# IvanIZ/BenchPush

Hardware: AMD Instinct MI355X
Metric: env-steps/sec at N=4096 envs (ship-ice-v0), 1/2/4/8 MI355X (higher is better)
Workload: dtype f64

## Files before the change

### __graft_entry__.py

```python
import os
import subprocess
import sys

ROOT = os.path.dirname(os.path.abspath(__file__))
if ROOT not in sys.path:
    sys.path.insert(0, ROOT)


def build():
    from benchpush_amd.build import build_debug_paths, build_hip
    build_hip(force=True, verbose=True)
    build_debug_paths(force=True, verbose=True)
    subprocess.check_call(["make", "-C", os.path.join(ROOT, "oracle")])
    import benchpush_amd
    from benchpush_amd import _lib
    L = _lib.load()
    for name in _lib.EXPORTS:
        getattr(L, name)
    assert L.bp_abi_version() == 11


def smoke():
    import numpy as np
    import torch

    from benchpush_amd.envs.ship_ice import BatchedShipIceEnv, default_trials
    from oracle.oracle import OracleShipIce

    trials = default_trials(0.3, 2, base_seed=7)
    env = BatchedShipIceEnv(4, cfg={"concentration": 0.3}, trials=trials, device="cuda:0")
    obs, info = env.reset()
    cfg = env.cfg
    orcs = [OracleShipIce(env.params, cfg.ship.vertices, cfg.ship.head, cfg.ship.tail) for _ in range(4)]
    oobs = [o.reset(trials[e % 2])[0] for e, o in enumerate(orcs)]
    assert all(np.array_equal(obs[e].cpu().numpy(), oobs[e]) for e in range(4)), "reset observation differs from oracle"
    rng = np.random.default_rng(0)
    for t in range(2):
        a = rng.uniform(-1, 1, 4).astype(np.float32).astype(np.float64)
        obs, rew, term, trunc, info = env.step(torch.from_numpy(a))
        bs = env.body_state().cpu().numpy()
        for e, o in enumerate(orcs):
            oo, orr, ot, oi = o.step(float(a[e]))
            nb = len(o.bodies())
            assert np.array_equal(bs[e, :nb], o.bodies()), "body state differs from oracle"
            assert np.array_equal(obs[e].cpu().numpy(), oo), "observation differs from oracle"
            assert float(rew[e]) == orr and bool(term[e]) == ot, "reward/termination differs from oracle"
    env.check_errors()
    env.close()
    from benchpush_amd import box_delivery_scenario as S
    from benchpush_amd.envs.box_delivery import BatchedBoxDeliveryEnv
    from oracle.oracle_bd import BD_INFO_KEYS, OracleBoxDelivery

    benv = BatchedBoxDeliveryEnv(2, num_trials=2, device="cuda:0")
    bobs, _ = benv.reset()
    borc = []
    for e in range(2):
        o = OracleBoxDelivery(S.box_delivery_physics_params(benv.cfg), dict(benv.bd_params), benv.cfg)
        assert np.array_equal(bobs[e].cpu().numpy(), o.reset(benv.trials[e])), "box-delivery reset observation differs from oracle"
        borc.append(o)
    acts = np.array([0.4, -0.7])
    bobs, brew, bterm, btrunc, binfo = benv.step(torch.from_numpy(acts))
    for e, o in enumerate(borc):
        oo, orr, ot, otr, oi = o.step(float(acts[e]))
        assert np.array_equal(bobs[e].cpu().numpy(), oo) and float(brew[e]) == orr, "box-delivery step differs from oracle"
        assert np.array_equal(binfo[e].cpu().numpy(), np.array([oi[k] for k in BD_INFO_KEYS])), "box-delivery info differs from oracle"
    benv.check_errors()
    benv.close()
    print("smoke ok: ship-ice 4 envs x 2 steps and box-delivery 2 envs x 1 step bit-identical to the oracles")


if __name__ == "__main__":
    build()
    if len(sys.argv) > 1 and sys.argv[1] == "smoke":
        smoke()
```

### benchpush_amd/build.py

```python
import os
import subprocess

_HERE = os.path.dirname(os.path.abspath(__file__))
CSRC = os.path.join(_HERE, "csrc")
LIB_PATH = os.path.join(_HERE, "libbenchpush_hip.so")
SOURCES = ["bp_capi.hip"]


def _headers():
    import glob
    return sorted(glob.glob(os.path.join(CSRC, "*.hpp"))) + [os.path.join(_HERE, "..", "include", "benchpush_amd.h")]

HIPCC_FLAGS = ["--offload-arch=gfx950", "-O3", "-ffp-contract=off", "-fno-fast-math", "-fPIC", "-shared", "-std=c++17",
               "-Wno-unused-value"]


def needs_build():
    if not os.path.exists(LIB_PATH):
        return True
    t = os.path.getmtime(LIB_PATH)
    for p in [os.path.join(CSRC, f) for f in SOURCES] + _headers():
        if os.path.exists(p) and os.path.getmtime(p) > t:
            return True
    return False


def build_hip(force=False, verbose=False):
    if not force and not needs_build():
        return LIB_PATH
    hipcc = os.environ.get("HIPCC", "/opt/rocm/bin/hipcc")
    if not os.path.exists(hipcc):
        hipcc = "hipcc"
    cmd = [hipcc] + HIPCC_FLAGS + ["-o", LIB_PATH] + [os.path.join(CSRC, s) for s in SOURCES]
    if verbose:
        print(" ".join(cmd))
    subprocess.check_call(cmd, cwd=CSRC)
    return LIB_PATH


DBG_LIB_PATH = os.path.join(_HERE, "libbenchpush_hip_dbgpaths.so")


def build_debug_paths(force=False, verbose=False):
    if not force and os.path.exists(DBG_LIB_PATH):
        t = os.path.getmtime(DBG_LIB_PATH)
        if all(os.path.getmtime(p) <= t for p in [os.path.join(CSRC, f) for f in SOURCES] + _headers() if os.path.exists(p)):
            return DBG_LIB_PATH
    hipcc = os.environ.get("HIPCC", "/opt/rocm/bin/hipcc")
    if not os.path.exists(hipcc):
        hipcc = "hipcc"
    cmd = [hipcc] + HIPCC_FLAGS + ["-DBP_DEBUG_PATHS=1", "-o", DBG_LIB_PATH] + [os.path.join(CSRC, s) for s in SOURCES]
    if verbose:
        print(" ".join(cmd))
    subprocess.check_call(cmd, cwd=CSRC)
    return DBG_LIB_PATH


if __name__ == "__main__":
    print(build_hip(force=True, verbose=True))
    print(build_debug_paths(force=True, verbose=True))
```

### benchpush_amd/csrc/bp_capi.hip

```cpp
#include <hip/hip_runtime.h>

#include <cstdio>
#include <cstdlib>
#include <algorithm>
#include <cstring>
#include <map>
#include <mutex>
#include <string>
#include <vector>

#include <fcntl.h>
#include <sys/file.h>
#include <sys/stat.h>
#include <unistd.h>

#include "bp_host_bd.hpp"
#include "bp_boxdelivery.hpp"
#include "bp_policy.hpp"
#include "bp_render.hpp"

struct bp_handle {
    bp_config cfg;
    int num_envs = 0;
    long long env_offset = 0;
// ... 134 lines not shown
        L.fd = open(key.c_str(), O_RDWR | O_CREAT | O_CLOEXEC, 0666);
        umask(um);
        if (L.fd < 0) { g_res_locks.erase(key); return; }
        (void)flock(L.fd, LOCK_SH);
    }
    L.refs++;
    h->dev_lock_key = key;
}
static void resident_release(bp_handle *h)
{
    if (h->dev_lock_key.empty()) return;
    std::lock_guard<std::mutex> g(g_res_mu);
    auto it = g_res_locks.find(h->dev_lock_key);
    if (it != g_res_locks.end() && --it->second.refs <= 0) { close(it->second.fd); g_res_locks.erase(it); }
    h->dev_lock_key.clear();
}
static bool resident_device_shared(bp_handle *h)
{
    if (h->dev_lock_key.empty()) return false;
    std::lock_guard<std::mutex> g(g_res_mu);
    auto it = g_res_locks.find(h->dev_lock_key);
    if (it == g_res_locks.end()) return false;
    if (flock(it->second.fd, LOCK_EX | LOCK_NB) == 0) { (void)flock(it->second.fd, LOCK_SH); return false; }
    (void)flock(it->second.fd, LOCK_SH);
    return true;
}
static int device_cus(bp_handle *h)
{
    if (h->num_cus <= 0) {
        hipDeviceProp_t prop;
        HIPCHK(h, hipGetDeviceProperties(&prop, h->device));
        h->num_cus = prop.multiProcessorCount;
    }
    return BP_OK;
}
static int sched_persist_setup(bp_handle *h)
{
    int rc = device_cus(h);
    if (rc) return rc;
    const int slots = h->num_cus * 4 * (h->P.env_kind == BP_ENV_SHIP_ICE ? BP_SCHED_WAVES : 2);
    const int pers = getenv("BP_SCHED_PERSIST") ? atoi(getenv("BP_SCHED_PERSIST")) : 1;
    h->sched_persist = pers > 0 ? std::min(h->num_envs, slots * pers) : 0;
    if (h->sched_persist && !h->pd_buf) HIPCHK(h, hipMalloc(&h->pd_buf, sizeof(DevParams) + sizeof(DevPtrs)));
    if (h->sched_persist && !getenv("BP_SCHED_PERSIST")) {
        h->resident_auto = true;
        resident_acquire(h);
        h->device_shared = resident_device_shared(h);
    }
    return BP_OK;
}
extern "C" {

int32_t bp_abi_version(void) { return BP_ABI_VERSION; }
int32_t bp_sizeof_config(void) { return (int32_t)sizeof(bp_config); }

const char *bp_last_error(const bp_handle *h) { return h ? h->err.c_str() : "null handle"; }

int bp_create(const bp_config *cfg, int32_t num_envs, int64_t env_id_offset, int32_t device, bp_handle **out)
{
    if (!cfg || !out || num_envs <= 0) return BP_EINVAL;
    *out = nullptr;
    int ndev = 0;
    if (hipGetDeviceCount(&ndev) != hipSuccess || ndev <= 0 || device < 0 || device >= ndev) return BP_ENODEVICE;
    if (!(cfg->damping_pow >= 0.0) || cfg->damping_pow > 1.0) return BP_EINVAL;
    if (cfg->num_ship_verts < 3 || cfg->num_ship_verts > BP_MAX_SHIP_VERTS) return BP_EINVAL;
    if (cfg->steps <= 0 || cfg->iterations <= 0 || cfg->persistence <= 0) return BP_EINVAL;
    if (cfg->env_kind != BP_ENV_SHIP_ICE && cfg->env_kind != BP_ENV_MAZE) return BP_EINVAL;
    if (cfg->env_kind == BP_ENV_MAZE && (cfg->num_wheels < 0 || cfg->num_wheels > BP_MAX_WHEELS)) return BP_EINVAL;
    if (cfg->random_start && cfg->env_kind != BP_ENV_SHIP_ICE) return BP_EINVAL;
    bp_handle *h = new bp_handle();
    h->cfg = *cfg;
    h->num_envs = num_envs;
    h->env_offset = env_id_offset;
    h->device = device;
    h->resettle = (cfg->env_kind == BP_ENV_SHIP_ICE && cfg->random_start != 0);
    DevGuard _dg(device);
    if (!_dg.ok) { delete h; return BP_ENODEVICE; }
    memset(&h->D, 0, sizeof(h->D));
    DevParams &P = h->P;
    memset(&P, 0, sizeof(P));
    P.dt_sub = cfg->dt / cfg->steps;
    P.steps = cfg->steps; P.iterations = cfg->iterations; P.persistence = cfg->persistence; P.settle_steps = cfg->settle_steps;
    if (const char *evp = getenv("BP_DEBUG_PATHS")) P.dbg_paths = atoi(evp);
    P.damping_pow = cfg->damping_pow; P.bias_coef = cfg->bias_coef; P.slop = cfg->slop;
    P.target_speed = cfg->target_speed; P.max_yaw_rate = cfg->max_yaw_rate;
    P.map_w = cfg->map_w; P.map_h = cfg->map_h; P.goal_y = cfg->goal_y; P.m_to_pix = cfg->m_to_pix;
    P.beta = cfg->beta; P.boundary_penalty = cfg->boundary_penalty; P.terminal_reward = cfg->terminal_reward;
    P.local_w = cfg->local_w; P.local_h = cfg->local_h; P.vshift = cfg->vshift; P.obs_range = cfg->obs_range;
    P.skin = 0.06;
    P.env_kind = cfg->env_kind;
    P.nkin = (cfg->env_kind == BP_ENV_MAZE) ? 1 + cfg->num_wheels : 1;
    P.goal_x = cfg->goal_x; P.goal_reach = cfg->goal_reach; P.k_increment = cfg->k_increment;
    P.num_envs = num_envs; P.env_offset = env_id_offset;
    P.random_start = (cfg->env_kind == BP_ENV_SHIP_ICE) ? cfg->random_start : 0;
    P.start_x_range = cfg->start_x_range; P.start_seed = cfg->start_seed; P.ship_mass = cfg->ship_mass;
    P.num_ship_verts = cfg->num_ship_verts;
    memcpy(P.ship_verts, cfg->ship_verts, sizeof(P.ship_verts));
    memcpy(P.ship_head, cfg->ship_head, sizeof(P.ship_head));
    memcpy(P.ship_tail, cfg->ship_tail, sizeof(P.ship_tail));
    const double grid = 1.0 / cfg->m_to_pix;
    P.grid_w = (int)(cfg->map_w / grid);
    P.grid_h = (int)(cfg->map_h / grid);
    P.obs_h = (int)(cfg->local_h * cfg->m_to_pix);
    P.obs_w = (int)(cfg->local_w * cfg->m_to_pix);
    if ((P.obs_h * P.obs_w) % 4 != 0) { delete h; return BP_EINVAL; }
    if (cfg->env_kind == BP_ENV_MAZE) {
        const int infl = (P.obs_w > P.obs_h ? P.obs_w : P.obs_h) / 2;
        const int nwords = ((P.obs_h + infl) * (P.obs_w + infl) + 31) / 32;
        h->obs_lds_bytes = (size_t)4 * (nwords + ((nwords + 1) & ~1)) + sizeof(double) * 2 * MZ_MAXBOX * 4;
        if (hipFuncSetAttribute((const void *)k_observe_maze, hipFuncAttributeMaxDynamicSharedMemorySize, (int)h->obs_lds_bytes) != hipSuccess) { delete h; return BP_EHIP; }
    } else {
        if (P.obs_h % 2 != 0 || P.obs_w % 2 != 0 || P.obs_w / 2 > OBS_THREADS_SHIP) { delete h; return BP_EINVAL; }
        h->obs_lds_bytes = (size_t)((P.obs_h * P.obs_w + 15) & ~15) + (size_t)((P.obs_h + 15) & ~15) + sizeof(double) * 2 * OBS_CHUNK * BP_MAXV;
        if (hipFuncSetAttribute((const void *)k_observe, hipFuncAttributeMaxDynamicSharedMemorySize, (int)h->obs_lds_bytes) != hipSuccess) { delete h; return BP_EHIP; }
    }
    *out = h;
    return BP_OK;
}

int bp_destroy(bp_handle *h)
{
    if (!h) return BP_EINVAL;
    DevGuard _dg(h->device);
    if (h->st_aux) { hipStreamSynchronize(h->st_aux); hipStreamDestroy(h->st_aux); }
    resident_release(h);
    if (h->pd_buf) hipFree(h->pd_buf);
    if (h->st_aux2) { hipStreamSynchronize(h->st_aux2); hipStreamDestroy(h->st_aux2); }
    if (h->st_aux3) { hipStreamSynchronize(h->st_aux3); hipStreamDestroy(h->st_aux3); }
    if (h->ev_join3) hipEventDestroy(h->ev_join3);
    for (hipStream_t s_ : h->st_parts) { hipStreamSynchronize(s_); hipStreamDestroy(s_); }
    for (hipEvent_t e_ : h->ev_parts) hipEventDestroy(e_);
    if (h->ev_join2) hipEventDestroy(h->ev_join2);
    if (h->ev_fork) hipEventDestroy(h->ev_fork);
    if (h->ev_join) hipEventDestroy(h->ev_join);
    for (void *p : h->allocs) hipFree(p);
    for (hipEvent_t e : h->ev) hipEventDestroy(e);
    delete h;
    return BP_OK;
}

static int upload_trials(bp_handle *h, const std::vector<std::vector<bpgeom::Shape>> &trials, bool settle = true)
{
    using namespace bpgeom;
    const int T = (int)trials.size();
    int maxnb = 1;
    for (const auto &b : trials) maxnb = std::max(maxnb, (int)b.size());
    if (maxnb > 60000) return fail(h, BP_EINVAL, "too many bodies");
    const int nbcap = (maxnb + 7) / 8 * 8;
    h->nbcap = nbcap;
    h->num_trials = T;
    h->P.nbcap = nbcap;
    h->P.mvcap = mvcap_for(nbcap);
    h->P.num_trials = T;
    h->lds_bytes = lds_bytes_for(nbcap, h->P.env_kind == BP_ENV_BOX);
    if (h->lds_bytes > 160 * 1024) return fail(h, BP_EINVAL, "nb_cap too large for LDS");
    if (nbcap >= (1 << BP_CC_IDX_BITS)) return fail(h, BP_EINVAL, "nb_cap exceeds the candidate cache's body-index field (16384 bodies per env)");

    std::vector<int> h_nb(T), h_nv((size_t)T * nbcap, 0), h_kind((size_t)T * nbcap, 0);
    std::vector<d2> h_lv((size_t)T * nbcap * BP_MAXV), h_ln((size_t)T * nbcap * BP_MAXV);
    std::vector<double4> h_mass((size_t)T * nbcap), h_pose((size_t)T * nbcap), h_prop((size_t)T * nbcap);
    memset(h_lv.data(), 0, h_lv.size() * sizeof(d2));
    memset(h_ln.data(), 0, h_ln.size() * sizeof(d2));
    memset(h_mass.data(), 0, h_mass.size() * sizeof(double4));
    memset(h_pose.data(), 0, h_pose.size() * sizeof(double4));
    memset(h_prop.data(), 0, h_prop.size() * sizeof(double4));
    for (int t = 0; t < T; t++) {
// ... 833 lines not shown
{
    if (!h || !mask || !src || !dst || rows < 0 || row_bytes <= 0 || (row_bytes & 3) != 0 || rows > 0x7FFFFFFF) return BP_EINVAL;
    if ((((size_t)src) | ((size_t)dst)) & 3) return BP_EINVAL;
    BP_DEVICE(h);
    if (rows == 0) return BP_OK;
    hipLaunchKernelGGL(k_copy_rows_masked, dim3((unsigned)rows), dim3(256), 0, (hipStream_t)stream, (const unsigned char *)mask, (const unsigned *)src,
                       (unsigned *)dst, (long long)(row_bytes / 4));
    HIPCHK(h, hipGetLastError());
    return BP_OK;
}

int bp_debug_round2(const double *in_dev, double *out_dev, int32_t n, void *stream)
{
    if (!in_dev || !out_dev || n < 0) return BP_EINVAL;
    hipLaunchKernelGGL(k_debug_round2, dim3((n + 255) / 256), dim3(256), 0, (hipStream_t)stream, in_dev, out_dev, n);
    return hipGetLastError() == hipSuccess ? BP_OK : BP_EHIP;
}

int bp_get_body_state(bp_handle *h, double *out, void *stream)
{
    if (!h || !out) return BP_EINVAL;
    if (!h->loaded || !h->was_reset) return fail(h, BP_ESTATE, "not reset");
    BP_DEVICE(h);
    hipLaunchKernelGGL(k_export_bodies, dim3(h->num_envs), dim3(256), 0, (hipStream_t)stream, h->P, h->D, out);
    HIPCHK(h, hipGetLastError());
    return BP_OK;
}
int bp_costmap_update(bp_handle *h, const bp_costmap_config *cfg, const double *ship_pos_y, double vs, double *out, void *stream)
{
    if (!h || !cfg || !out) return BP_EINVAL;
    if (!h->loaded || !h->was_reset) return fail(h, BP_ESTATE, "bp_costmap_update before bp_load_scenarios/bp_reset");
    if (h->P.env_kind != BP_ENV_SHIP_ICE) return fail(h, BP_EINVAL, "bp_costmap_update: ship-ice handles only");
    const int H = (int)(cfg->m * cfg->scale), W = (int)(cfg->n * cfg->scale);
    if (!(cfg->scale > 0) || H <= 0 || W <= 0 || cfg->margin < 0 || 2 * cfg->margin > W) return fail(h, BP_EINVAL, "bp_costmap_update: bad grid");
    BP_DEVICE(h);
    hipStream_t st = (hipStream_t)stream;
    const size_t total = (size_t)h->num_envs * H * W;
    const int nblk = (int)std::min<size_t>((total + 255) / 256, 65535);
    hipLaunchKernelGGL(k_costmap_init, dim3(nblk), dim3(256), 0, st, out, h->num_envs, H, W, (int)cfg->margin);
    const int groups = (h->P.nbcap - h->P.nkin + 3) / 4;
    if (groups > 0)
        hipLaunchKernelGGL(k_costmap, dim3(h->num_envs, groups), dim3(256), 0, st, h->P, h->D, cfg->scale, H, W, cfg->alpha, cfg->ship_mass,
                           cfg->horizon > 0 ? cfg->horizon * cfg->scale : 0.0, ship_pos_y, vs, out);
    HIPCHK(h, hipGetLastError());
    return BP_OK;
}
int bp_get_low_dim_obs(bp_handle *h, double *out, void *stream)
{
    if (!h || !out) return BP_EINVAL;
    if (!h->loaded || !h->was_reset) return fail(h, BP_ESTATE, "not reset");
    BP_DEVICE(h);
    hipLaunchKernelGGL(k_export_lowdim, dim3(h->num_envs), dim3(256), 0, (hipStream_t)stream, h->P, h->D, out);
    HIPCHK(h, hipGetLastError());
    return BP_OK;
}

int32_t bp_nb_cap(const bp_handle *h) { return h ? h->nbcap : 0; }
int32_t bp_obs_height(const bp_handle *h) { return h ? h->P.obs_h : 0; }
int32_t bp_obs_width(const bp_handle *h) { return h ? h->P.obs_w : 0; }

int32_t bp_bd_sizeof_config(void) { return (int32_t)sizeof(bp_bd_config); }

int bp_bd_create(const bp_bd_config *cfg, int32_t num_envs, int64_t env_id_offset, int32_t device, bp_handle **out)
{
    if (!cfg || !out || num_envs <= 0) return BP_EINVAL;
    *out = nullptr;
    int ndev = 0;
    if (hipGetDeviceCount(&ndev) != hipSuccess || ndev <= 0 || device < 0 || device >= ndev) return BP_ENODEVICE;
    if (!(cfg->damping_pow >= 0.0) || cfg->damping_pow > 1.0 || cfg->steps <= 0 || cfg->iterations <= 0 || cfg->persistence <= 0) return BP_EINVAL;
    if (cfg->num_boxes <= 0 || cfg->num_boxes > BD_MAXBOX || cfg->local_px <= 0 || (cfg->local_px & 1)) return BP_EINVAL;
    bp_handle *h = new bp_handle();
    memset(&h->cfg, 0, sizeof(h->cfg));
    h->bdcfg = *cfg;
    h->num_envs = num_envs; h->env_offset = env_id_offset; h->device = device;
    DevGuard _dg(device);
    if (!_dg.ok) { delete h; return BP_ENODEVICE; }
    memset(&h->D, 0, sizeof(h->D));
    memset(&h->Q, 0, sizeof(h->Q));
    DevParams &P = h->P;
    memset(&P, 0, sizeof(P));
    P.dt_sub = cfg->ctrl_dt / cfg->steps;
    P.steps = cfg->steps; P.iterations = cfg->iterations; P.persistence = cfg->persistence; P.settle_steps = cfg->settle_steps;
    if (const char *evp = getenv("BP_DEBUG_PATHS")) P.dbg_paths = atoi(evp);
    P.damping_pow = cfg->damping_pow; P.bias_coef = cfg->bias_coef; P.slop = cfg->slop;
    P.target_speed = cfg->target_speed;
    P.skin = 0.25;
    P.env_kind = BP_ENV_BOX;
    P.nkin = 6;
    P.num_envs = num_envs; P.env_offset = env_id_offset;
    P.obs_h = P.obs_w = cfg->local_px;
    BdParams &B = h->B;
    memset(&B, 0, sizeof(B));
    B.room_length = cfg->room_length; B.room_width = cfg->room_width; B.recept_x = cfg->recept_x; B.recept_y = cfg->recept_y;
    B.recept_size = cfg->recept_size; B.ppm = cfg->ppm; B.local_w = cfg->local_w; B.robot_radius = cfg->robot_radius;
    B.step_size = cfg->step_size; B.target_speed = cfg->target_speed; B.ctrl_dt = cfg->ctrl_dt;
    B.partial_rewards_scale = cfg->partial_rewards_scale; B.goal_reward = cfg->goal_reward; B.collision_penalty = cfg->collision_penalty;
    B.non_movement_penalty = cfg->non_movement_penalty; B.correct_direction_reward_scale = cfg->correct_direction_reward_scale;
    B.ministep_size = cfg->ministep_size; B.sp_channel_scale = cfg->sp_channel_scale;
    B.local_px = cfg->local_px; B.use_correct_direction_reward = cfg->use_correct_direction_reward;
    B.inactivity_cutoff = cfg->inactivity_cutoff; B.num_boxes = cfg->num_boxes; B.step_limit = cfg->step_limit;
    B.first_box = 6;
    B.action_type = cfg->action_type;
    if (cfg->action_type < 0 || cfg->action_type > 2) { delete h; return BP_EINVAL; }
    B.task = cfg->task; B.omega_scale = cfg->omega_scale; B.v_scale = cfg->v_scale; B.lfc = cfg->lfc;
    B.yaw_rate_step = cfg->yaw_rate_step; B.t_max = cfg->t_max;
    B.boundary_penalty = cfg->boundary_penalty; B.box_cleared_reward = cfg->box_cleared_reward; B.box_putback_penalty = cfg->box_putback_penalty;
    B.truncation_penalty = cfg->truncation_penalty; B.terminal_reward = cfg->terminal_reward; B.pushing_mult = cfg->pushing_mult;
    B.recept_outside = (cfg->task == 0 && cfg->invert_receptacle_map) ? 1.0f : 0.0f;
    if (cfg->task == 1) {
        if (cfg->num_boundary_verts < 3 || cfg->num_boundary_verts > 8 || cfg->num_outer_verts < 3 || cfg->num_outer_verts > 8 ||
            cfg->num_goal_points < 1 || cfg->num_goal_points > 128) { delete h; return BP_EINVAL; }
        B.nbd = cfg->num_boundary_verts; B.nob = cfg->num_outer_verts; B.ngoal = cfg->num_goal_points;
        memcpy(B.bd_poly, cfg->boundary, sizeof(B.bd_poly)); memcpy(B.ob_poly, cfg->outer_boundary, sizeof(B.ob_poly));
        memcpy(B.footprint, cfg->footprint_verts, sizeof(B.footprint));
        B.recept_outside = 1.0f;
    } else if (cfg->task != 0) { delete h; return BP_EINVAL; }
    *out = h;
    return BP_OK;
}

int bp_bd_load(bp_handle *h, int32_t T, int32_t nbox, const double *starts, const double *boxes, int32_t ns, const double *sverts,
               const int32_t *scount, const double *spose, const double *srad, const int32_t *stype)
{
    if (!h || T <= 0 || nbox <= 0 || nbox > BD_MAXBOX || ns <= 0 || !starts || !boxes || !sverts || !scount || !spose || !srad || !stype) return BP_EINVAL;
    if (h->loaded) return fail(h, BP_ESTATE, "scenarios already loaded");
    if (h->P.env_kind != BP_ENV_BOX) return fail(h, BP_ESTATE, "handle was created for another environment");
    BP_DEVICE(h);
    using namespace bpgeom;
    const bp_bd_config &cf = h->bdcfg;
    std::vector<std::vector<Shape>> trials(T);
    std::vector<Shape> recepts(T);
    h->bd_map_of_trial.assign(T, 0);
    std::vector<std::vector<std::vector<P2>>> map_keys;
    int nphys_static = -1;
    for (int t = 0; t < T; t++) {
        std::vector<Shape> &bodies = trials[t];
        const double sx = starts[3 * t], sy = starts[3 * t + 1], sh = starts[3 * t + 2];
        {
            Shape s;
            build_agent_main(cf.robot_verts, 4, sx, sy, sh, s);
            s.radius = 0.0; s.e = 0.01; s.u = 1.0; s.kind = kind_of(1, 1, BODY_KINEMATIC);
            bodies.push_back(s);
            for (int k = 0; k < 5; k++) {
                Shape w;
                build_kinematic_part(k < 4 ? cf.wheel_verts[k] : cf.bumper_verts, 4, sx, sy, sh, w);
                w.radius = 0.02; w.e = 0.01; w.u = 0.0; w.kind = kind_of(0, 1, BODY_KINEMATIC);
                bodies.push_back(w);
            }
        }
        for (int b = 0; b < nbox; b++) {
            const double *bx = boxes + ((size_t)t * nbox + b) * 3;
            Shape s;
            if (!build_box(bx[0], bx[1], bx[2], cf.box_half, cf.box_density, 0.02, s)) return fail(h, BP_EINVAL, "degenerate box");
            s.radius = 0.02; s.e = 0.01; s.u = 1.0; s.kind = kind_of(2, 0, BODY_DYNAMIC);
            bodies.push_back(s);
        }
        std::vector<std::vector<P2>> obstacles;
        int nrec = 0, nst = 0;
        for (int k = 0; k < ns; k++) {
            const size_t o = (size_t)t * ns + k;
            const int n = scount[o];
            if (n == 0) continue;
            if (n < 3 || n > 4) return fail(h, BP_EINVAL, "static polygons have 3 or 4 vertices");
            Shape s;
            build_static_poly(sverts + o * 8, n, spose[o * 3], spose[o * 3 + 1], spose[o * 3 + 2], s);
            s.radius = srad[o]; s.e = 0.01; s.u = 1.0;
// ... 462 lines not shown
```

### benchpush_amd/csrc/bp_device.hpp

```cpp
#pragma once
#include <hip/hip_runtime.h>
#include <stdint.h>

#include "../../include/benchpush_amd.h"

#define BP_KADJ 24
#define BP_ACAP 64

typedef double2 d2;

enum { BODY_DYNAMIC = 0, BODY_KINEMATIC = 1, BODY_STATIC = 2 };
__device__ __forceinline__ int kind_ctype(int k) { return k & 0xFF; }
__device__ __forceinline__ int kind_group(int k) { return (k >> 8) & 0xFF; }
__device__ __forceinline__ int kind_btype(int k) { return (k >> 16) & 3; }
enum { ARB_FIRST = 0, ARB_NORMAL = 1, ARB_IGNORE = 2, ARB_CACHED = 3 };
#define ARB_FREE_KEY 0xFFFFFFFFu

struct DevParams {
    double dt_sub;
    int steps, iterations, persistence, settle_steps;
    double damping_pow, bias_coef, slop, target_speed, max_yaw_rate, map_w, map_h, goal_y, m_to_pix;
    double beta, boundary_penalty, terminal_reward, local_w, local_h, vshift, obs_range;
    double goal_x, goal_reach, k_increment;
    int env_kind;
    int nkin;
    double skin;
    int nbcap, mvcap, num_envs, num_trials, num_ship_verts;
    long long env_offset;
    double ship_verts[BP_MAX_SHIP_VERTS][2];
    double ship_head[2], ship_tail[2];
    int obs_h, obs_w, grid_h, grid_w;
    int sq_chunk, sq_levels, sq_cap;
    int sq_cls;
    unsigned sq_ymask;
    int sq_dynprio;
    int sq_parts, sq_part;
    int sq_floor;
    int sq_lrpt, sq_bw, sq_hyst;
    int sq_hold;
    int sq_mode;
    int sq_image;
    unsigned sq_img_lds;
    unsigned sq_img_stride;
    int sq_debug;
    int dbg_paths;
    int pair_mode, pair_solo;
    int pp_max_keys, pp_max_slots, pp_max_mv, pp_max_act, pp_max_work;
    int pp_snake, pp_heavy_only;
    int pp_rate;
    int random_start;
    double start_x_range, ship_mass;
    unsigned long long start_seed;
};

struct DevPtrs {
    const int *sc_nb;
    const int *sc_nv;
    const d2 *sc_lv;
    const d2 *sc_ln;
    const double4 *sc_mass;
    const double4 *sc_pose;
    const double4 *sc_prop;
    const int *sc_kind;
    const double *dist_map;
    const unsigned char *wall_map;
    const double *goal_raw;
    const double *maze_obs_map;
    int *e_trial, *e_episode, *e_nb, *e_err;
    int *e_flags;
    double *e_prevdist;
    unsigned *e_stamp;
    double *e_currdt, *e_total_work, *e_ke, *e_imp;
    unsigned *e_cnt;
    unsigned *e_cost;
    const int *order;
    int *sq_items;
    int *sq_ctr;
    unsigned *sq_carry;
    unsigned char *sq_moved;
    unsigned char *sq_img;
    int *sq_done;
    int *sq_lev;
    unsigned *sq_thr;
    int *sq_sub;
    int *sq_pairstat;
    int *sq_rescue;
    int *sq_warn;
    d2 *pxy;
    double *ang;
    d2 *rot;
    d2 *velv, *velw, *velb;
    d2 *wv, *wn, *pv;
    double4 *bb, *fat;
    unsigned short *adj;
    unsigned char *adjn;
    unsigned long long *hint;
    unsigned *a_key, *a_stamp, *a_sc, *a_h0, *a_h1;
    double *a_d;
    double *e_lastrew;
    int *e_lastflag;
    double *m_acc;
    double *m_rows;
    double *m_ring;
    double *m_sum;
    unsigned *m_count;
    unsigned char *m_open;
    unsigned long long *clk;
    double *dbg;
    int dbg_env;
    unsigned long long *prof;
};

__device__ __forceinline__ d2 mk2(double x, double y) { d2 r; r.x = x; r.y = y; return r; }
__device__ __forceinline__ double vdot(d2 a, d2 b) { return a.x * b.x + a.y * b.y; }
__device__ __forceinline__ double vcross(d2 a, d2 b) { return a.x * b.y - a.y * b.x; }
__device__ __forceinline__ d2 vsub(d2 a, d2 b) { return mk2(a.x - b.x, a.y - b.y); }
__device__ __forceinline__ d2 vadd(d2 a, d2 b) { return mk2(a.x + b.x, a.y + b.y); }
__device__ __forceinline__ d2 vneg(d2 a) { return mk2(-a.x, -a.y); }
__device__ __forceinline__ d2 vmul(d2 a, double s) { return mk2(a.x * s, a.y * s); }
__device__ __forceinline__ d2 vperp(d2 a) { return mk2(-a.y, a.x); }
__device__ __forceinline__ d2 vrotate(d2 a, d2 b) { return mk2(a.x * b.x - a.y * b.y, a.x * b.y + a.y * b.x); }
__device__ __forceinline__ double vlen(d2 a) { return __builtin_sqrt(vdot(a, a)); }
__device__ __forceinline__ d2 vlerp(d2 a, d2 b, double t) { return vadd(vmul(a, 1.0 - t), vmul(b, t)); }
__device__ __forceinline__ double clamp01(double f) { return fmax(0.0, fmin(f, 1.0)); }
__device__ __forceinline__ double fclampd(double f, double lo, double hi) { return fmin(fmax(f, lo), hi); }

#define HW_PLANE_A(h) ((int)((h) & 31ull))
// ... 92 lines not shown
__device__ __forceinline__ void bp_sincos(double x, double &sn, double &cs)
{
    const double invpio2 = 6.36619772367581382433e-01;
    const double pio2_1 = 1.57079632673412561417e+00, pio2_1t = 6.07710050650619224932e-11;
    const double pio2_2 = 6.07710050630396597660e-11, pio2_2t = 2.02226624879595063154e-21;
    const double S1 = -1.66666666666666324348e-01, S2 = 8.33333333332248946124e-03, S3 = -1.98412698298579493134e-04,
                 S4 = 2.75573137070700676789e-06, S5 = -2.50507602534068634195e-08, S6 = 1.58969099521155010221e-10;
    const double C1 = 4.16666666666666019037e-02, C2 = -1.38888888888741095749e-03, C3 = 2.48015872894767294178e-05,
                 C4 = -2.75573143513906633035e-07, C5 = 2.08757232129817482790e-09, C6 = -1.13596475577881948265e-11;
    double fn = __builtin_rint(x * invpio2);
    double r = x - fn * pio2_1;
    double w = fn * pio2_1t;
    double y0 = r - w;
    const bool deep = __builtin_fabs(y0) < __builtin_fabs(x) * 7.62939453125e-06;
    if (__builtin_expect(__ballot(deep) != 0ull, 0)) {
        const double t = r;
        const double w2 = fn * pio2_2;
        const double r2 = t - w2;
        const double w3 = fn * pio2_2t - ((t - r2) - w2);
        if (deep) { r = r2; w = w3; y0 = r2 - w3; }
    }
    double y1 = (r - y0) - w;
    int q = (int)((long long)fn & 3);
    double z = y0 * y0;
    double v = z * y0;
    double rs = S2 + z * (S3 + z * (S4 + z * (S5 + z * S6)));
    double ks = y0 - ((z * (0.5 * y1 - v * rs) - y1) - v * S1);
    double rc = z * (C1 + z * (C2 + z * (C3 + z * (C4 + z * (C5 + z * C6)))));
    double kc = 1.0 - (0.5 * z - (z * rc - y0 * y1));
    const bool odd = (q & 1) != 0;
    const double s0 = odd ? kc : ks, c0 = odd ? ks : kc;
    const int sflip = (q & 2) ? (int)0x80000000 : 0, cflip = ((q + 1) & 2) ? (int)0x80000000 : 0;
    sn = __hiloint2double(__double2hiint(s0) ^ sflip, __double2loint(s0));
    cs = __hiloint2double(__double2hiint(c0) ^ cflip, __double2loint(c0));
}

__host__ __device__ inline unsigned long long bp_splitmix64(unsigned long long x)
{
    x += 0x9E3779B97F4A7C15ull;
    x = (x ^ (x >> 30)) * 0xBF58476D1CE4E5B9ull;
    x = (x ^ (x >> 27)) * 0x94D049BB133111EBull;
    return x ^ (x >> 31);
}
__host__ __device__ inline double bp_start_u01(unsigned long long seed, long long gid, long long episode)
{
    const unsigned long long k = bp_splitmix64(seed ^ bp_splitmix64(((unsigned long long)gid << 32) + (unsigned long long)episode));
    return (double)(k >> 11) * (1.0 / 9007199254740992.0);
}

__device__ __forceinline__ int lane_id() { return (int)(threadIdx.x & 63); }
__device__ __forceinline__ unsigned long long ballot(bool p) { return __ballot(p); }
__device__ __forceinline__ int popc_below(unsigned long long m, int lane) { return __popcll(m & ((1ull << lane) - 1ull)); }

template <int CTRL>
__device__ __forceinline__ double dpp_mov_f64(double v)
{
    int lo = __double2loint(v), hi = __double2hiint(v);
    lo = __builtin_amdgcn_update_dpp(lo, lo, CTRL, 0xF, 0xF, false);
    hi = __builtin_amdgcn_update_dpp(hi, hi, CTRL, 0xF, 0xF, false);
    return __hiloint2double(hi, lo);
}
__device__ __forceinline__ double half_max(double v)
{
    v = fmax(v, dpp_mov_f64<0xB1>(v));
    v = fmax(v, dpp_mov_f64<0x4E>(v));
    v = fmax(v, dpp_mov_f64<0x141>(v));
    v = fmax(v, dpp_mov_f64<0x140>(v));
    v = fmax(v, __shfl_xor(v, 16));
    return v;
}
__device__ __forceinline__ double half_min(double v)
{
    v = fmin(v, dpp_mov_f64<0xB1>(v));
    v = fmin(v, dpp_mov_f64<0x4E>(v));
    v = fmin(v, dpp_mov_f64<0x141>(v));
    v = fmin(v, dpp_mov_f64<0x140>(v));
    v = fmin(v, __shfl_xor(v, 16));
    return v;
}
__device__ __forceinline__ double readlane_f64(double v, int l)
{
    return __hiloint2double(__builtin_amdgcn_readlane(__double2hiint(v), l), __builtin_amdgcn_readlane(__double2loint(v), l));
}
__device__ __forceinline__ void halves_max_f64(double v, double &lo, double &hi)
{
    v = fmax(v, dpp_mov_f64<0xB1>(v));
    v = fmax(v, dpp_mov_f64<0x4E>(v));
    v = fmax(v, dpp_mov_f64<0x141>(v));
    v = fmax(v, dpp_mov_f64<0x140>(v));
    lo = fmax(readlane_f64(v, 0), readlane_f64(v, 16));
    hi = fmax(readlane_f64(v, 32), readlane_f64(v, 48));
}
__device__ __forceinline__ double oct_min_f64(double v)
{
    double p;
    p = dpp_mov_f64<0xB1>(v); v = (p < v) ? p : v;
    p = dpp_mov_f64<0x4E>(v); v = (p < v) ? p : v;
    p = dpp_mov_f64<0x141>(v); v = (p < v) ? p : v;
    return v;
}
__device__ __forceinline__ int oct_min_i32(int v)
{
    v = min(v, __builtin_amdgcn_update_dpp(v, v, 0xB1, 0xF, 0xF, false));
    v = min(v, __builtin_amdgcn_update_dpp(v, v, 0x4E, 0xF, 0xF, false));
    v = min(v, __builtin_amdgcn_update_dpp(v, v, 0x141, 0xF, 0xF, false));
    return v;
}
__device__ __forceinline__ unsigned long long f64_key(double v)
{
    const unsigned long long b = __builtin_bit_cast(unsigned long long, v);
    return (b >> 63) ? ~b : (b | 0x8000000000000000ull);
}
__device__ __forceinline__ double key_f64(unsigned long long k)
{
    const unsigned long long b = (k >> 63) ? (k & 0x7FFFFFFFFFFFFFFFull) : ~k;
    return __builtin_bit_cast(double, b);
}
__device__ __forceinline__ void lds_sync() { asm volatile("" ::: "memory"); }
```

### benchpush_amd/csrc/bp_physics.hpp

```cpp
#pragma once
#include "bp_device.hpp"
#include <type_traits>

#ifdef BP_PROF
#define PROF_DECL unsigned long long _pt = __builtin_amdgcn_s_memtime();
#define PROF_ACC(slot) { unsigned long long _n = __builtin_amdgcn_s_memtime(); if (lane_id() == 0) L.prof[slot] += _n - _pt; _pt = _n; }
#define PROF_CNT(slot, v) { const unsigned long long _v = (unsigned long long)(v); if (lane_id() == 0) L.prof[slot] += _v; }
#define PROF_MAX(slot, v) { const unsigned long long _v = (unsigned long long)(v); if (lane_id() == 0 && _v > L.prof[slot]) L.prof[slot] = _v; }
#else
#define PROF_DECL
#define PROF_ACC(slot)
#define PROF_CNT(slot, v)
#define PROF_MAX(slot, v)
#endif


#define BP_UNLIKELY(x) __builtin_expect(!!(x), 0)
#define BP_UNLIKELY2(x) __builtin_expect(!!(x), 0)
#ifdef BP_DEBUG_PATHS
#define BP_DBGP(bit) ((P.dbg_paths & (bit)) != 0)
#define BP_TRACE_ON(D) ((D).dbg != nullptr)
#else
#define BP_DBGP(bit) false
#define BP_TRACE_ON(D) false
// ... 933 lines not shown
    const bool any_bias = ballot(warm && ((bias0 != 0.0) || (A.count > 1 && bias1 != 0.0))) != 0;
    if (BP_UNLIKELY(amask != S.prev_amask)) {
        PROF_CNT(41, 1)
        int rank = 0;
        unsigned long long m = amask;
        while (m) {
            const int l = __ffsll((long long)m) - 1;
            m &= m - 1;
            const unsigned k = (unsigned)__builtin_amdgcn_readlane((int)A.key, l);
            rank += (k < A.key) ? 1 : 0;
        }
        A.rank = rank;
        lds_sync();
        if (active) { L.colmask[A.slotA] = 0; L.colmask[A.slotB] = 0; }
        lds_sync();
        const int nact = __popcll(amask);
        int nlev = 0;
        for (int r = 0; r < nact; r++) {
            const unsigned long long rm = ballot(active && A.rank == r);
            const int l = __ffsll((long long)rm) - 1;
            const bool adyn = __builtin_amdgcn_readlane(__double2hiint(A.ma), l) != 0 || __builtin_amdgcn_readlane(__double2loint(A.ma), l) != 0;
            const bool bdyn = __builtin_amdgcn_readlane(__double2hiint(A.mb), l) != 0 || __builtin_amdgcn_readlane(__double2loint(A.mb), l) != 0;
            const int a = __builtin_amdgcn_readlane(A.slotA, l), b = __builtin_amdgcn_readlane(A.slotB, l);
            const unsigned ua = adyn ? (unsigned)L.colmask[a] : 0u, ub = bdyn ? (unsigned)L.colmask[b] : 0u;
            const unsigned used = ua | ub;
            int c = __ffs(~used) - 1;
            if (c > 15) { c = 15; S.err |= BP_ERR_LEVEL_OVERFLOW; }
            if (adyn) L.colmask[a] = (unsigned short)(ua | (1u << c));
            if (bdyn) L.colmask[b] = (unsigned short)(ub | (1u << c));
            if (lane == l) A.level = c + 1;
            nlev = max(nlev, c + 1);
        }
        S.nlevels = nlev;
        S.prev_amask = amask;
    }
    PROF_CNT(21, __popcll(wmask))
    PROF_MAX(13, __popcll(wmask))
    S.costp += 16u + 2u * (unsigned)__popcll(amask) + 4u * (unsigned)(__popcll(wmask) * S.nlevels);
    lds_sync();
    if (DAMP) {
        for (int s0 = 0; s0 < S.nslots; s0 += 64) {
            const int sl = s0 + lane;
            if (sl >= P.nkin && sl < S.nslots) {
                const d2 v = L.sv[sl], w2 = L.sw[sl];
                L.sv[sl] = mk2(v.x * P.damping_pow + 0.0, v.y * P.damping_pow + 0.0);
                L.sw[sl] = mk2(w2.x * P.damping_pow + 0.0, w2.y);
            }
        }
    } else
    for (int k0 = 0; k0 < S.nmv; k0 += 64) {
        const int k = k0 + lane;
        if (k < S.nmv) {
            const int i = L.mv[k];
            const int sl = L.slot_of[i];
            if (sl != 255 && i >= P.nkin) { L.sv[sl] = mk2(0.0, 0.0); L.sw[sl].x = 0.0; }
        }
    }
    lds_sync();
    PROF_ACC(6)
    const double dt_coef = (prev_dt == 0.0) ? 0.0 : (prev_dt == dt) ? 1.0 : dt / prev_dt;
    const int nlevels = wmask ? S.nlevels : 0;
    unsigned lvlmask = 0;
    for (int lvl = 1; lvl <= nlevels; lvl++) if (ballot(warm && A.level == lvl)) lvlmask |= 1u << lvl;
    for (unsigned lm = lvlmask; lm; lm &= lm - 1u) {
        const int lvl = __ffs((int)lm) - 1;
        if (warm && A.level == lvl && A.state != ARB_FIRST) {
            d2 va = L.sv[A.slotA], vb = L.sv[A.slotB];
            double wa = L.sw[A.slotA].x, wb = L.sw[A.slotB].x;
            {
                const d2 j = vmul(vrotate(A.n, mk2(A.jn0, A.jt0)), dt_coef);
                apply_contact_impulses(A, 0, va, wa, vb, wb, j);
            }
            if (A.count > 1) {
                const d2 j = vmul(vrotate(A.n, mk2(A.jn1, A.jt1)), dt_coef);
                apply_contact_impulses(A, 1, va, wa, vb, wb, j);
            }
            if (A.ma != 0.0) { L.sv[A.slotA] = va; L.sw[A.slotA].x = wa; }
            if (A.mb != 0.0) { L.sv[A.slotB] = vb; L.sw[A.slotB].x = wb; }
        }
        lds_sync();
    }
    PROF_ACC(7)
    constexpr bool SCRATCH_WB = (KIND != BP_ENV_BOX);
    const int wA = (!SCRATCH_WB || A.ma != 0.0) ? A.slotA : BP_NSLOT, wB = (!SCRATCH_WB || A.mb != 0.0) ? A.slotB : BP_NSLOT;
    auto iterate = [&](auto bias_tag) {
    constexpr bool AB = decltype(bias_tag)::value;
    auto gather = [&](d2 &va, d2 &vb, d2 &wa2, d2 &wb2, d2 &vba, d2 &vbb) {
        va = L.sv[A.slotA]; vb = L.sv[A.slotB];
        wa2 = mk2(0.0, 0.0); wb2 = mk2(0.0, 0.0); vba = mk2(0.0, 0.0); vbb = mk2(0.0, 0.0);
        if (AB) { wa2 = L.sw[A.slotA]; wb2 = L.sw[A.slotB]; vba = L.sb[A.slotA]; vbb = L.sb[A.slotB]; }
        else { wa2.x = L.sw[A.slotA].x; wb2.x = L.sw[A.slotB].x; }
    };
    auto scatter = [&](const d2 va, const d2 vb, const d2 wa2, const d2 wb2, const d2 vba, const d2 vbb) {
        if (SCRATCH_WB) {
            L.sv[wA] = va; if (AB) { L.sw[wA] = wa2; L.sb[wA] = vba; } else L.sw[wA].x = wa2.x;
            L.sv[wB] = vb; if (AB) { L.sw[wB] = wb2; L.sb[wB] = vbb; } else L.sw[wB].x = wb2.x;
        } else {
            if (A.ma != 0.0) { L.sv[A.slotA] = va; if (AB) { L.sw[A.slotA] = wa2; L.sb[A.slotA] = vba; } else L.sw[A.slotA].x = wa2.x; }
            if (A.mb != 0.0) { L.sv[A.slotB] = vb; if (AB) { L.sw[A.slotB] = wb2; L.sb[A.slotB] = vbb; } else L.sw[A.slotB].x = wb2.x; }
        }
    };
    auto contacts = [&](d2 &va, d2 &vb, d2 &wa2, d2 &wb2, d2 &vba, d2 &vbb, double &chg) {
        const d2 n = A.n;
#pragma unroll
        for (int c = 0; c < 2; c++) {
            if (c == 0 || A.count > 1) {
                const d2 r1 = c ? A.r1_1 : A.r1_0, r2 = c ? A.r2_1 : A.r2_0;
                const double nMass = c ? nMass1 : nMass0, tMass = c ? tMass1 : tMass0;
                const double bias = c ? bias1 : bias0, bounce = c ? bounce1 : bounce0;
                const d2 v1 = vadd(va, vmul(vperp(r1), wa2.x));
                const d2 v2 = vadd(vb, vmul(vperp(r2), wb2.x));
                const d2 vr = vsub(v2, v1);
                const double vrn = vdot(vr, n);
                const double vrt = vdot(vr, vperp(n));
                const double jbnOld = c ? jBias1 : jBias0;
                double jBias = jbnOld;
                if (AB) {
                    const d2 vb1 = vadd(vba, vmul(vperp(r1), wa2.y));
                    const d2 vb2 = vadd(vbb, vmul(vperp(r2), wb2.y));
                    const double vbn = vdot(vsub(vb2, vb1), n);
                    const double jbn = (bias - vbn) * nMass;
                    jBias = fmax(jbnOld + jbn, 0.0);
                }
                const double jn = -(bounce + vrn) * nMass;
                const double jnOld = c ? A.jn1 : A.jn0;
                const double jnAcc = fmax(jnOld + jn, 0.0);
                const double jtMax = A.u * jnAcc;
                const double jt = -vrt * tMass;
                const double jtOld = c ? A.jt1 : A.jt0;
                const double jtAcc = fclampd(jtOld + jt, -jtMax, jtMax);
                if (c) { jBias1 = jBias; A.jn1 = jnAcc; A.jt1 = jtAcc; }
                else   { jBias0 = jBias; A.jn0 = jnAcc; A.jt0 = jtAcc; }
                if (AB) {
                    const double djb = jBias - jbnOld;
                    chg += __builtin_fabs(djb);
                    const d2 jb = vmul(n, djb);
                    const d2 jbneg = vneg(jb);
                    vba = vadd(vba, vmul(jbneg, A.ma));
                    wa2.y += A.ia * vcross(r1, jbneg);
                    vbb = vadd(vbb, vmul(jb, A.mb));
                    wb2.y += A.ib * vcross(r2, jb);
                }
                const double djn = jnAcc - jnOld, djt = jtAcc - jtOld;
                chg += __builtin_fabs(djn); chg += __builtin_fabs(djt);
                const d2 j = vrotate(n, mk2(djn, djt));
                apply_contact_impulses(A, c, va, wa2.x, vb, wb2.x, j);
            }
        }
    };
    if (!AB && KIND != BP_ENV_BOX && (lvlmask & (lvlmask - 1u)) == 0u && lvlmask != 0u) {
        d2 va = mk2(0.0, 0.0), vb = va, wa2 = va, wb2 = va, vba = va, vbb = va;
        if (warm) gather(va, vb, wa2, wb2, vba, vbb);
        auto negzero = [](double x) { return (((unsigned)__double2hiint(x) ^ 0x80000000u) | (unsigned)__double2loint(x)) == 0u; };
        bool nz = false;
        if (warm && A.ma == 0.0) nz = negzero(va.x) || negzero(va.y) || negzero(wa2.x) || (AB && (negzero(wa2.y) || negzero(vba.x) || negzero(vba.y)));
        if (warm && A.mb == 0.0) nz = nz || negzero(vb.x) || negzero(vb.y) || negzero(wb2.x) || (AB && (negzero(wb2.y) || negzero(vbb.x) || negzero(vbb.y)));
        if (!ballot(nz)) {
            for (int it = 0; it < P.iterations; it++) {
                PROF_CNT(42, 1)
                PROF_CNT(43, 1)
                double chg = 0.0;
                if (warm) contacts(va, vb, wa2, wb2, vba, vbb, chg);
                if (BP_UNLIKELY2(!ballot(warm && chg != 0.0))) break;
            }
            if (warm) scatter(va, vb, wa2, wb2, vba, vbb);
            lds_sync();
            return;
        }
    }
    for (int it = 0; it < P.iterations; it++) {
        PROF_CNT(42, 1)
        double chg = 0.0;
        for (unsigned lm = lvlmask; lm; lm &= lm - 1u) {
            const int lvl = __ffs((int)lm) - 1;
            PROF_CNT(43, 1)
            PROF_CNT(44, ballot(warm && A.level == lvl && A.count > 1) ? 1 : 0)
            if (warm && A.level == lvl) {
                d2 va, vb, wa2, wb2, vba, vbb;
                gather(va, vb, wa2, wb2, vba, vbb);
                contacts(va, vb, wa2, wb2, vba, vbb, chg);
                scatter(va, vb, wa2, wb2, vba, vbb);
            }
            lds_sync();
        }
        if (BP_UNLIKELY2(!ballot(warm && chg != 0.0))) break;
    }
    };
    if (any_bias) iterate(std::true_type{}); else iterate(std::false_type{});
    PROF_ACC(8)
    {
        const bool shiparb = active && ba == 0;
        const unsigned long long sm = ballot(shiparb);
        S.ship_post = (unsigned)__popcll(sm);
        S.ship_contacts = (unsigned)__popcll(sm) + (unsigned)__popcll(ballot(shiparb && A.count > 1));
        if (sm) {
            S.n_post += (unsigned)__popcll(sm);
            S.n_contact += (unsigned)__popcll(sm) + (unsigned)__popcll(ballot(shiparb && A.count > 1));
            S.n_first += (unsigned)__popcll(ballot(shiparb && A.state == ARB_FIRST));
            const bool ws = shiparb && warm;
            const unsigned long long wsm = ballot(ws);
            if (wsm) {
                const double e_first = readlane_f64(A.e, __ffsll((long long)wsm) - 1);
                double eCoef;
                if (!ballot(ws && A.e != e_first)) {
                    if (e_first != S.ecoef_e) { S.ecoef_e = e_first; S.ecoef = (1 - e_first) / (1 + e_first); }
                    eCoef = S.ecoef;
                } else eCoef = (1 - A.e) / (1 + A.e);
                double ke = 0.0;
                d2 js = mk2(0.0, 0.0);
                if (ws) {
                    ke += eCoef * A.jn0 * A.jn0 / nMass0 + A.jt0 * A.jt0 / tMass0;
                    js = vadd(js, vrotate(A.n, mk2(A.jn0, A.jt0)));
                    if (A.count > 1) {
                        ke += eCoef * A.jn1 * A.jn1 / nMass1 + A.jt1 * A.jt1 / tMass1;
                        js = vadd(js, vrotate(A.n, mk2(A.jn1, A.jt1)));
                    }
                }
                const double imp = vlen(js);
                const int ns = __popcll(sm);
                for (int r = 0; r < ns; r++) {
                    const unsigned long long rm = ballot(ws && A.rank == r);
                    if (!rm) continue;
                    const int l = __ffsll((long long)rm) - 1;
                    S.total_ke += readlane_f64(ke, l);
                    S.total_imp += readlane_f64(imp, l);
                }
            }
        }
    }
    if (ship_rules) {
        const double a0 = L.ag[0].x;
        const double x0 = L.sp[0].x;
        if (KIND == BP_ENV_SHIP_ICE && ship_rules == 1 && (a0 <= 0.0 || a0 >= BP_PI)) {
            if (lane < P.nkin) L.sw[lane] = mk2(0.0, L.sw[lane].y);
            S.yaw_violated = 1;
        }
        if (x0 < 0.0 || x0 > P.map_w) S.boundary_violated = 1;
    }
    lds_sync();
    {
        bool wantA = false, wantB = false;
        if (active) {
            if (A.ma != 0.0) {
                const d2 v = L.sv[A.slotA], w2 = L.sw[A.slotA], vb = L.sb[A.slotA];
                wantA = (v.x != 0.0 || v.y != 0.0 || w2.x != 0.0 || w2.y != 0.0 || vb.x != 0.0 || vb.y != 0.0);
            }
            if (A.mb != 0.0) {
                const d2 v = L.sv[A.slotB], w2 = L.sw[A.slotB], vb = L.sb[A.slotB];
                wantB = (v.x != 0.0 || v.y != 0.0 || w2.x != 0.0 || w2.y != 0.0 || vb.x != 0.0 || vb.y != 0.0);
            }
            if (KIND == BP_ENV_BOX) {
                if (A.ma != 0.0 && ((S.evmask >> ba) & 1ull)) wantA = true;
                if (A.mb != 0.0 && ((S.evmask >> bbi) & 1ull)) wantB = true;
            }
        }
        const d2 v0 = L.sv[0], w0 = L.sw[0];
        const int shipmv = (KIND == BP_ENV_BOX || v0.x != 0.0 || v0.y != 0.0 || w0.x != 0.0) ? P.nkin : 0;
        bool differs = false;
        if (lane < shipmv) { differs = L.mv[lane] != (unsigned short)lane; L.mv[lane] = (unsigned short)lane; }
        int nA_ = 0;
        unsigned long long mB = 0ull;
        if (DAMP) {
            int pos0 = shipmv;
            for (int s0 = 0; s0 < S.nslots; s0 += 64) {
                const int sl = s0 + lane;
                bool want = false;
                unsigned short body = 0;
                if (sl >= P.nkin && sl < S.nslots) {
                    body = L.sbody[sl];
                    const d2 v = L.sv[sl], w2 = L.sw[sl], vb = L.sb[sl];
                    want = (v.x != 0.0 || v.y != 0.0 || w2.x != 0.0 || w2.y != 0.0 || vb.x != 0.0 || vb.y != 0.0);
// ... 29 lines not shown
```

Measured before the change: 271,900.

## Solve bias impulses on mirrored free lanes instead of the combined bias path

```diff
diff --git a/__graft_entry__.py b/__graft_entry__.py
--- a/__graft_entry__.py
+++ b/__graft_entry__.py
@@ -8,9 +8,10 @@
 
 
 def build():
-    from benchpush_amd.build import build_debug_paths, build_hip
+    from benchpush_amd.build import build_debug_paths, build_hip, build_prof
     build_hip(force=True, verbose=True)
     build_debug_paths(force=True, verbose=True)
+    build_prof(force=True, verbose=True)
     subprocess.check_call(["make", "-C", os.path.join(ROOT, "oracle")])
     import benchpush_amd
     from benchpush_amd import _lib
diff --git a/benchpush_amd/build.py b/benchpush_amd/build.py
--- a/benchpush_amd/build.py
+++ b/benchpush_amd/build.py
@@ -56,6 +56,25 @@
     return DBG_LIB_PATH
 
 
+PROF_LIB_PATH = os.path.join(_HERE, "libbenchpush_hip_prof.so")
+
+
+def build_prof(force=False, verbose=False):
+    if not force and os.path.exists(PROF_LIB_PATH):
+        t = os.path.getmtime(PROF_LIB_PATH)
+        if all(os.path.getmtime(p) <= t for p in [os.path.join(CSRC, f) for f in SOURCES] + _headers() if os.path.exists(p)):
+            return PROF_LIB_PATH
+    hipcc = os.environ.get("HIPCC", "/opt/rocm/bin/hipcc")
+    if not os.path.exists(hipcc):
+        hipcc = "hipcc"
+    cmd = [hipcc] + HIPCC_FLAGS + ["-DBP_PROF=1", "-o", PROF_LIB_PATH] + [os.path.join(CSRC, s) for s in SOURCES]
+    if verbose:
+        print(" ".join(cmd))
+    subprocess.check_call(cmd, cwd=CSRC)
+    return PROF_LIB_PATH
+
+
 if __name__ == "__main__":
     print(build_hip(force=True, verbose=True))
     print(build_debug_paths(force=True, verbose=True))
+    print(build_prof(force=True, verbose=True))
diff --git a/benchpush_amd/csrc/bp_capi.hip b/benchpush_amd/csrc/bp_capi.hip
--- a/benchpush_amd/csrc/bp_capi.hip
+++ b/benchpush_amd/csrc/bp_capi.hip
@@ -240,6 +240,7 @@
     P.dt_sub = cfg->dt / cfg->steps;
     P.steps = cfg->steps; P.iterations = cfg->iterations; P.persistence = cfg->persistence; P.settle_steps = cfg->settle_steps;
     if (const char *evp = getenv("BP_DEBUG_PATHS")) P.dbg_paths = atoi(evp);
+    P.bias_lanes = getenv("BP_BIAS_LANES") ? (atoi(getenv("BP_BIAS_LANES")) != 0) : 1;
     P.damping_pow = cfg->damping_pow; P.bias_coef = cfg->bias_coef; P.slop = cfg->slop;
     P.target_speed = cfg->target_speed; P.max_yaw_rate = cfg->max_yaw_rate;
     P.map_w = cfg->map_w; P.map_h = cfg->map_h; P.goal_y = cfg->goal_y; P.m_to_pix = cfg->m_to_pix;
@@ -1239,6 +1240,7 @@
     P.dt_sub = cfg->ctrl_dt / cfg->steps;
     P.steps = cfg->steps; P.iterations = cfg->iterations; P.persistence = cfg->persistence; P.settle_steps = cfg->settle_steps;
     if (const char *evp = getenv("BP_DEBUG_PATHS")) P.dbg_paths = atoi(evp);
+    P.bias_lanes = getenv("BP_BIAS_LANES") ? (atoi(getenv("BP_BIAS_LANES")) != 0) : 1;
     P.damping_pow = cfg->damping_pow; P.bias_coef = cfg->bias_coef; P.slop = cfg->slop;
     P.target_speed = cfg->target_speed;
     P.skin = 0.25;
diff --git a/benchpush_amd/csrc/bp_device.hpp b/benchpush_amd/csrc/bp_device.hpp
--- a/benchpush_amd/csrc/bp_device.hpp
+++ b/benchpush_amd/csrc/bp_device.hpp
@@ -43,6 +43,7 @@
     unsigned sq_img_lds;
     unsigned sq_img_stride;
     int sq_debug;
+    int bias_lanes;
     int dbg_paths;
     int pair_mode, pair_solo;
     int pp_max_keys, pp_max_slots, pp_max_mv, pp_max_act, pp_max_work;
@@ -301,6 +302,10 @@
 {
     return __hiloint2double(__builtin_amdgcn_readlane(__double2hiint(v), l), __builtin_amdgcn_readlane(__double2loint(v), l));
 }
+__device__ __forceinline__ double bperm_f64(int lane4, double v)
+{
+    return __hiloint2double(__builtin_amdgcn_ds_bpermute(lane4, __double2hiint(v)), __builtin_amdgcn_ds_bpermute(lane4, __double2loint(v)));
+}
 __device__ __forceinline__ void halves_max_f64(double v, double &lo, double &hi)
 {
     v = fmax(v, dpp_mov_f64<0xB1>(v));
diff --git a/benchpush_amd/csrc/bp_physics.hpp b/benchpush_amd/csrc/bp_physics.hpp
--- a/benchpush_amd/csrc/bp_physics.hpp
+++ b/benchpush_amd/csrc/bp_physics.hpp
@@ -1039,19 +1039,56 @@
     }
     PROF_ACC(7)
     constexpr bool SCRATCH_WB = (KIND != BP_ENV_BOX);
+    constexpr bool MIRRORS = (KIND != BP_ENV_BOX);
+    bool solve = warm;
+    bool mirrored = false;
+    bool mir = false;
+    if (MIRRORS && any_bias) {
+        PROF_CNT(45, 1)
+        const unsigned long long fmask = ballot(A.key == ARB_FREE_KEY);
+        const int nw = __popcll(wmask);
+        if (P.bias_lanes != 0 && __popcll(fmask) >= nw) {
+            PROF_CNT(46, 1)
+            PROF_CNT(48, (lvlmask & (lvlmask - 1u)) != 0u ? 1 : 0)
+            mirrored = true;
+            if (warm) L.owner[popc_below(wmask, lane)] = (unsigned short)lane;
+            lds_sync();
+            const int fr = popc_below(fmask, lane);
+            mir = (A.key == ARB_FREE_KEY) && fr < nw;
+            const int src4 = (mir ? (int)L.owner[fr] : lane) << 2;
+            lds_sync();
+            auto take = [&](double &f) { const double t = bperm_f64(src4, f); if (mir) f = t; };
+            take(A.n.x); take(A.n.y);
+            take(A.r1_0.x); take(A.r1_0.y); take(A.r2_0.x); take(A.r2_0.y);
+            take(A.r1_1.x); take(A.r1_1.y); take(A.r2_1.x); take(A.r2_1.y);
+            take(A.ma); take(A.ia); take(A.mb); take(A.ib);
+            take(nMass0); take(nMass1);
+            const double b0 = bperm_f64(src4, bias0), b1 = bperm_f64(src4, bias1);
+            const int packed = __builtin_amdgcn_ds_bpermute(src4, A.count | (A.level << 8) | (A.slotA << 16) | (A.slotB << 24));
+            if (mir) {
+                A.count = packed & 0xFF; A.level = (packed >> 8) & 0xFF; A.slotA = (packed >> 16) & 0xFF; A.slotB = (packed >> 24) & 0xFF;
+                bounce0 = -b0; bounce1 = -b1; tMass0 = 0.0; tMass1 = 0.0;
+                A.jn0 = A.jt0 = A.jn1 = A.jt1 = 0.0; A.u = 0.0;
+            }
+            solve = warm || mir;
+        } else { PROF_CNT(47, 1) }
+    }
+    d2 *const gvA = (mir ? L.sb : L.sv) + A.slotA, *const gvB = (mir ? L.sb : L.sv) + A.slotB;
+    double *const gwA = &L.sw[A.slotA].x + (mir ? 1 : 0), *const gwB = &L.sw[A.slotB].x + (mir ? 1 : 0);
     const int wA = (!SCRATCH_WB || A.ma != 0.0) ? A.slotA : BP_NSLOT, wB = (!SCRATCH_WB || A.mb != 0.0) ? A.slotB : BP_NSLOT;
+    d2 *const svA = (mir ? L.sb : L.sv) + wA, *const svB = (mir ? L.sb : L.sv) + wB;
+    double *const swA = &L.sw[wA].x + (mir ? 1 : 0), *const swB = &L.sw[wB].x + (mir ? 1 : 0);
     auto iterate = [&](auto bias_tag) {
     constexpr bool AB = decltype(bias_tag)::value;
     auto gather = [&](d2 &va, d2 &vb, d2 &wa2, d2 &wb2, d2 &vba, d2 &vbb) {
-        va = L.sv[A.slotA]; vb = L.sv[A.slotB];
         wa2 = mk2(0.0, 0.0); wb2 = mk2(0.0, 0.0); vba = mk2(0.0, 0.0); vbb = mk2(0.0, 0.0);
-        if (AB) { wa2 = L.sw[A.slotA]; wb2 = L.sw[A.slotB]; vba = L.sb[A.slotA]; vbb = L.sb[A.slotB]; }
-        else { wa2.x = L.sw[A.slotA].x; wb2.x = L.sw[A.slotB].x; }
+        if (AB) { va = L.sv[A.slotA]; vb = L.sv[A.slotB]; wa2 = L.sw[A.slotA]; wb2 = L.sw[A.slotB]; vba = L.sb[A.slotA]; vbb = L.sb[A.slotB]; }
+        else { va = *gvA; vb = *gvB; wa2.x = *gwA; wb2.x = *gwB; }
     };
     auto scatter = [&](const d2 va, const d2 vb, const d2 wa2, const d2 wb2, const d2 vba, const d2 vbb) {
         if (SCRATCH_WB) {
-            L.sv[wA] = va; if (AB) { L.sw[wA] = wa2; L.sb[wA] = vba; } else L.sw[wA].x = wa2.x;
-            L.sv[wB] = vb; if (AB) { L.sw[wB] = wb2; L.sb[wB] = vbb; } else L.sw[wB].x = wb2.x;
+            if (AB) { L.sv[wA] = va; L.sw[wA] = wa2; L.sb[wA] = vba; } else { *svA = va; *swA = wa2.x; }
+            if (AB) { L.sv[wB] = vb; L.sw[wB] = wb2; L.sb[wB] = vbb; } else { *svB = vb; *swB = wb2.x; }
         } else {
             if (A.ma != 0.0) { L.sv[A.slotA] = va; if (AB) { L.sw[A.slotA] = wa2; L.sb[A.slotA] = vba; } else L.sw[A.slotA].x = wa2.x; }
             if (A.mb != 0.0) { L.sv[A.slotB] = vb; if (AB) { L.sw[A.slotB] = wb2; L.sb[A.slotB] = vbb; } else L.sw[A.slotB].x = wb2.x; }
@@ -1107,20 +1144,20 @@
     };
     if (!AB && KIND != BP_ENV_BOX && (lvlmask & (lvlmask - 1u)) == 0u && lvlmask != 0u) {
         d2 va = mk2(0.0, 0.0), vb = va, wa2 = va, wb2 = va, vba = va, vbb = va;
-        if (warm) gather(va, vb, wa2, wb2, vba, vbb);
+        if (solve) gather(va, vb, wa2, wb2, vba, vbb);
         auto negzero = [](double x) { return (((unsigned)__double2hiint(x) ^ 0x80000000u) | (unsigned)__double2loint(x)) == 0u; };
         bool nz = false;
-        if (warm && A.ma == 0.0) nz = negzero(va.x) || negzero(va.y) || negzero(wa2.x) || (AB && (negzero(wa2.y) || negzero(vba.x) || negzero(vba.y)));
-        if (warm && A.mb == 0.0) nz = nz || negzero(vb.x) || negzero(vb.y) || negzero(wb2.x) || (AB && (negzero(wb2.y) || negzero(vbb.x) || negzero(vbb.y)));
+        if (solve && A.ma == 0.0) nz = negzero(va.x) || negzero(va.y) || negzero(wa2.x) || (AB && (negzero(wa2.y) || negzero(vba.x) || negzero(vba.y)));
+        if (solve && A.mb == 0.0) nz = nz || negzero(vb.x) || negzero(vb.y) || negzero(wb2.x) || (AB && (negzero(wb2.y) || negzero(vbb.x) || negzero(vbb.y)));
         if (!ballot(nz)) {
             for (int it = 0; it < P.iterations; it++) {
                 PROF_CNT(42, 1)
                 PROF_CNT(43, 1)
                 double chg = 0.0;
-                if (warm) contacts(va, vb, wa2, wb2, vba, vbb, chg);
-                if (BP_UNLIKELY2(!ballot(warm && chg != 0.0))) break;
-            }
-            if (warm) scatter(va, vb, wa2, wb2, vba, vbb);
+                if (solve) contacts(va, vb, wa2, wb2, vba, vbb, chg);
+                if (BP_UNLIKELY2(!ballot(solve && chg != 0.0))) break;
+            }
+            if (solve) scatter(va, vb, wa2, wb2, vba, vbb);
             lds_sync();
             return;
         }
@@ -1131,8 +1168,8 @@
         for (unsigned lm = lvlmask; lm; lm &= lm - 1u) {
             const int lvl = __ffs((int)lm) - 1;
             PROF_CNT(43, 1)
-            PROF_CNT(44, ballot(warm && A.level == lvl && A.count > 1) ? 1 : 0)
-            if (warm && A.level == lvl) {
+            PROF_CNT(44, ballot(solve && A.level == lvl && A.count > 1) ? 1 : 0)
+            if (solve && A.level == lvl) {
                 d2 va, vb, wa2, wb2, vba, vbb;
                 gather(va, vb, wa2, wb2, vba, vbb);
                 contacts(va, vb, wa2, wb2, vba, vbb, chg);
@@ -1140,10 +1177,10 @@
             }
             lds_sync();
         }
-        if (BP_UNLIKELY2(!ballot(warm && chg != 0.0))) break;
+        if (BP_UNLIKELY2(!ballot(solve && chg != 0.0))) break;
     }
     };
-    if (any_bias) iterate(std::true_type{}); else iterate(std::false_type{});
+    if (any_bias && !mirrored) iterate(std::true_type{}); else iterate(std::false_type{});
     PROF_ACC(8)
     {
         const bool shiparb = active && ba == 0;
```

New measurement: 289,700, median of 6. 6.5% higher.
